# Gepeng18/Sentinel

Hardware: AMD Instinct MI355X
Metric: admission decisions/sec at 1M rules Zipf(1.1), 1/2/4/8 GPU; % HBM peak (higher is better)
Workload: dtype int64

## Files before the change

sentinel_amd/csrc/cluster.hip:

```cpp
#include "cluster.hpp"
#include "cluster_exact.hpp"
#include "cparam_exact.hpp"

#include <cstdio>
#include <cstdlib>

#include <algorithm>
#include <type_traits>

namespace sga {

namespace {

constexpr int kThreads = 256;
constexpr int kItems = 16;
constexpr int kTileElems = kThreads * kItems;

enum : uint8_t { RUN_FAST = 0, RUN_DONE = 1 };

__device__ __forceinline__ uint64_t lanemask_lt64(int lane) { return (1ULL << lane) - 1ULL; }

__device__ __forceinline__ HashEntry slot_lookup(const ClusterState &st, int64_t fid) {
    uint32_t h = (uint32_t)hash_flow_id(fid) & st.hmask;
    for (uint32_t probe = 0; probe <= st.hmask; ++probe) {
// ... 452 lines not shown
    const uint32_t f = pass_prefix(thr, P.isec, s0, a, n);
    uint32_t cpf = ri.cp_tot;
    if (f < n && ri.cp_tot > 0) cpf = prio_before(f);
    const uint32_t np_after = ri.cp_tot - cpf;
    uint32_t cw = 0;
    if (np_after > 0) {
        const int64_t w0 = c[CEV_WAITING] + waiting_others();
        const double latest = div_isec((double)(s0 + (int64_t)f * a), P.isec);
        const double lim = st.max_occupy_ratio * thr;
        const int64_t occ0 = o.occ_pass;
        uint32_t l2 = 0, h2 = np_after;
#pragma nounroll
        while (l2 < h2) {
            const uint32_t cc = l2 + ((h2 - l2) >> 1);
            const int64_t add = (int64_t)cc * a;
            const bool ok = (div_isec((double)(w0 + add), P.isec) <= lim) &&
                            (latest + (double)((int64_t)a + occ0 + add) - (double)head <= thr);
            if (ok) l2 = cc + 1;
            else h2 = cc;
        }
        cw = l2;
        if (cw > 0) {
            o.occ_pass += (int64_t)cw * a;
            o.occ_preq += cw;
            o.has_occ = 1;
            occ_dirty = true;
        }
    }
    const uint32_t nblk = n - f - cw;
    c[CEV_PASS] += (int64_t)f * a;
    c[CEV_PASS_REQUEST] += f;
    c[CEV_OCCUPIED_PASS] += (int64_t)cpf * a;
    c[CEV_WAITING] += (int64_t)cw * a;
    c[CEV_BLOCK] += (int64_t)nblk * a;
    c[CEV_BLOCK_REQUEST] += nblk;
    c[CEV_OCCUPIED_BLOCK] += (int64_t)(np_after - cw) * a;
    ro.s0 = s0;
    ro.thr = thr;
    ro.isec = P.isec;
    ro.f = f;
    ro.cpf = cpf;
    ro.cw = cw;
    ro.wait = (uint16_t)(1000 / P.S);
    ro.mode = RUN_FAST;
}

__device__ __forceinline__ void occ_transfer(int64_t (&c)[CEV_N], SlotOcc &o, bool &occ_dirty) {
    if (!o.has_occ) return;
    c[CEV_OCCUPIED_PASS] += o.occ_pass;
    c[CEV_PASS] += o.occ_pass;
    c[CEV_PASS_REQUEST] += o.occ_preq;
    o.occ_pass = 0;
    o.occ_preq = 0;
    o.has_occ = 0;
    occ_dirty = true;
}

template <class PrioBefore>
__device__ __forceinline__ bool run_compact(const ClusterState &st, const SlotParam &P, const Rec &R, double thr_in,
                                            bool hdr_thr, int64_t qbase, const RunIn &ri, PrioBefore prio_before,
                                            RunOut &ro, bool &wide) {
    int4 *lv = reinterpret_cast<int4 *>(R.ln());
    int4 L[8];
#pragma unroll
    for (int k = 0; k < 8; ++k) L[k] = lv[k];
    const uint64_t b0 = (uint64_t)i64_lo(L[LN_BASE / 4]);
    wide = (b0 & kLnWide) != 0;
    if (wide) return false;
    const int32_t a = ri.a;
    const int64_t q = qbase + ri.bd;
    if (a <= 0 || q < 0 || (int64_t)P.interval != (int64_t)P.S * (int64_t)P.W) return false;
    if (ri.cp_tot > 0 && (P.S <= 1 || 1000 / P.S <= 0)) return false;
    uint64_t b = b0;
    if (!(b & kLnBaseSet)) {
        const int64_t nb = ln_pick_base(q);
        if (!ln_base_fits(nb)) return false;
        b = (b & ~kLnBaseMask) | kLnBaseSet | (uint64_t)nb;
    }
    const int64_t base = ln_base(b);
    if (!ln_delta_fits(q, base)) return false;
    const uint32_t dq = ln_enc_delta(q, base);
    const int64_t qs = div_pos(q, P.S);
    const int cj = (int)(q - qs * P.S);
    const int jh = cj + 1 == P.S ? 0 : cj + 1;
    const double thr = hdr_thr ? f64_hi(L[LN_THR / 4]) : thr_in;
    auto valid = [&](uint32_t d) { return d != kLnNoBucket && !((int64_t)dq - (int64_t)d > (int64_t)P.S); };
    uint32_t dcur = kLnNoBucket, pcur = 0, dh = kLnNoBucket, ph = 0;
    int64_t bp = 0;
    auto take = [&](int jj, int d, int pv) {
        if (jj == cj) {
            dcur = (uint32_t)d;
            pcur = (uint32_t)pv;
        } else if (valid((uint32_t)d)) {
            bp += (int64_t)(uint32_t)pv;
        }
        if (jj == jh) {
            dh = (uint32_t)d;
            ph = (uint32_t)pv;
        }
    };
#pragma unroll
    for (int k = 0; k < kLnPairs / 2; ++k) {
        take(2 * k, L[k].x, L[k].y);
        take(2 * k + 1, L[k].z, L[k].w);
    }
    if (dcur != kLnNoBucket && dq < dcur) return false;
    const bool rot = dcur == kLnNoBucket || dq > dcur;
    int64_t c[CEV_N];
    SlotOcc o{(int64_t)(uint32_t)L[6].x, (int64_t)(uint32_t)L[6].y, (b & kLnHasOcc) ? 1 : 0, 0};
    bool occ_dirty = false;
    if (rot) {
#pragma unroll
        for (int k = 0; k < CEV_N; ++k) c[k] = 0;
        if (dcur != kLnNoBucket) occ_transfer(c, o, occ_dirty);
    } else {
        c[CEV_PASS] = (int64_t)pcur;
        if (ln_tag(b) == cj) {
            c[CEV_WAITING] = (int64_t)(uint32_t)L[6].z;
            c[CEV_BLOCK] = (int64_t)(uint32_t)L[6].w;
            c[CEV_PASS_REQUEST] = (int64_t)(uint32_t)L[7].x;
            c[CEV_BLOCK_REQUEST] = (int64_t)(uint32_t)L[7].y;
            c[CEV_OCCUPIED_PASS] = (int64_t)(uint32_t)L[7].z;
            c[CEV_OCCUPIED_BLOCK] = (int64_t)(uint32_t)L[7].w;
        } else {
            const int4 *cv = reinterpret_cast<const int4 *>(R.group(cj));
            const int4 c01 = cv[0], c23 = cv[1], c45 = cv[2];
            c[CEV_WAITING] = i64_lo(c01);
            c[CEV_BLOCK] = i64_hi(c01);
            c[CEV_PASS_REQUEST] = i64_lo(c23);
            c[CEV_BLOCK_REQUEST] = i64_hi(c23);
            c[CEV_OCCUPIED_PASS] = i64_lo(c45);
            c[CEV_OCCUPIED_BLOCK] = i64_hi(c45);
        }
    }
    const int64_t head = jh == cj ? c[CEV_PASS] : (valid(dh) ? (int64_t)ph : 0);
    auto waiting_others = [&]() {
        int64_t wv[kLnPairs], w0 = 0;
#pragma unroll
        for (int jj = 0; jj < kLnPairs; ++jj) wv[jj] = R.group(min(jj, P.S - 1))[0];
#pragma unroll
        for (int jj = 0; jj < kLnPairs; ++jj) {
            const uint32_t d = (uint32_t)((jj & 1) ? L[jj / 2].z : L[jj / 2].x);
            if (jj < P.S && jj != cj && valid(d)) w0 += wv[jj];
        }
        return w0;
    };
    run_decide(st, P, thr, ri, prio_before, waiting_others, bp, head, c, o, occ_dirty, ro);
    if (!ln_count_fits(c[CEV_PASS]) || !ln_count_fits(o.occ_pass) || !ln_count_fits(o.occ_preq)) return false;
    bool cfit = true;
#pragma unroll
    for (int k = 1; k < CEV_N; ++k) cfit = cfit && ln_count_fits(c[k]);
    uint64_t nb = ln_with_tag(b, cfit ? cj : -1);
    nb = o.has_occ ? (nb | kLnHasOcc) : (nb & ~kLnHasOcc);
    int4 pp = L[0];
#pragma unroll
    for (int k = 1; k < kLnPairs / 2; ++k)
        if (k == (cj >> 1)) pp = L[k];
    if (cj & 1) {
        pp.z = (int)dq;
        pp.w = (int)(uint32_t)c[CEV_PASS];
    } else {
        pp.x = (int)dq;
        pp.y = (int)(uint32_t)c[CEV_PASS];
    }
    lv[cj >> 1] = pp;
    if (nb != b0) lv[LN_BASE / 4] = make_int4((int)(uint32_t)nb, (int)(uint32_t)(nb >> 32), L[5].z, L[5].w);
    lv[6] = make_int4((int)(uint32_t)o.occ_pass, (int)(uint32_t)o.occ_preq, (int)(uint32_t)c[CEV_WAITING],
                      (int)(uint32_t)c[CEV_BLOCK]);
    lv[7] = make_int4((int)(uint32_t)c[CEV_PASS_REQUEST], (int)(uint32_t)c[CEV_BLOCK_REQUEST],
                      (int)(uint32_t)c[CEV_OCCUPIED_PASS], (int)(uint32_t)c[CEV_OCCUPIED_BLOCK]);
    int4 *cg = reinterpret_cast<int4 *>(R.group(cj));
    cg[0] = i4_of(c[CEV_WAITING], c[CEV_BLOCK]);
    cg[1] = i4_of(c[CEV_PASS_REQUEST], c[CEV_BLOCK_REQUEST]);
    cg[2] = i4_of(c[CEV_OCCUPIED_PASS], c[CEV_OCCUPIED_BLOCK]);
    return true;
}
static_assert(LN_BASE == 20 && LN_THR == 22 && LN_OCC == 24 && LN_CACHE == 26,
              "run_compact's pieces: 5 = (base word, threshold), 6 = (occupy counters, WAITING, BLOCK), 7 = the rest");

template <class PrioBefore>
__device__ __forceinline__ bool run_wide(const ClusterState &st, const SlotParam &P, const Rec &R, double thr_in,
                                         bool hdr_thr, int64_t qbase, const RunIn &ri, PrioBefore prio_before,
                                         RunOut &ro) {
    const int32_t a = ri.a;
    const int64_t q = qbase + ri.bd;
    const int64_t ws = q * P.W;
    const int64_t t0 = ws;
    const int64_t qs = div_pos(q, P.S);
    const int cj = (int)(q - qs * P.S);
    const int jh = cj + 1 == P.S ? 0 : cj + 1;
    const int4 *v = reinterpret_cast<const int4 *>(R.r);
    const int4 *hv = reinterpret_cast<const int4 *>(R.w_cache());
    const int4 *ov = reinterpret_cast<const int4 *>(&R.w_occ());
    const int4 o0 = ov[0], o1 = ov[1];
    int4 c01 = hv[0], c23 = hv[1], c45 = hv[2];
    const int4 meta = hv[3];
    const int4 cur = v[cj];
    const double thr = hdr_thr ? f64_hi(meta) : thr_in;
    auto valid = [&](int64_t w) { return w != kAbsent && !(t0 - w > (int64_t)P.interval); };
    int64_t bp = 0, hstart = kAbsent, hpass = 0;
    for (int jj = 0; jj < P.S; ++jj) {
        const int4 sp = v[jj];
        const int64_t w = i64_lo(sp), pv = i64_hi(sp);
        if (jj == jh) {
            hstart = w;
            hpass = pv;
        }
        if (jj != cj && valid(w)) bp += pv;
    }
    const int64_t old = i64_lo(cur);
    if (a <= 0 || (old != kAbsent && ws < old)) return false;
    if (ri.cp_tot > 0 && (P.S <= 1 || 1000 / P.S <= 0)) return false;
    const bool rot = old == kAbsent || ws > old;
    const bool tag_was_cur = i64_lo(meta) == old;
    if (!rot && !tag_was_cur) {
        const int4 *cv = reinterpret_cast<const int4 *>(R.group(cj));
        c01 = cv[0];
        c23 = cv[1];
        c45 = cv[2];
    }
    int64_t c[CEV_N];
    SlotOcc o{i64_lo(o0), i64_hi(o0), o1.x, o1.y};
    bool occ_dirty = false;
    if (rot) {
#pragma unroll
        for (int k = 0; k < CEV_N; ++k) c[k] = 0;
        if (old != kAbsent) occ_transfer(c, o, occ_dirty);
    } else {
        c[CEV_PASS] = i64_hi(cur);
        c[CEV_WAITING] = i64_lo(c01);
        c[CEV_BLOCK] = i64_hi(c01);
        c[CEV_PASS_REQUEST] = i64_lo(c23);
        c[CEV_BLOCK_REQUEST] = i64_hi(c23);
        c[CEV_OCCUPIED_PASS] = i64_lo(c45);
        c[CEV_OCCUPIED_BLOCK] = i64_hi(c45);
    }
    const int64_t head = jh == cj ? c[CEV_PASS] : (valid(hstart) ? hpass : 0);
    auto waiting_others = [&]() {
        int64_t w0 = 0;
#pragma nounroll
        for (int jj = 0; jj < P.S; ++jj)
            if (jj != cj && valid(R.w_start(jj))) w0 += R.cnt(CEV_WAITING, jj);
        return w0;
    };
    run_decide(st, P, thr, ri, prio_before, waiting_others, bp, head, c, o, occ_dirty, ro);
    const int64_t stv = rot ? ws : old;
    reinterpret_cast<int4 *>(R.r)[cj] = i4_of(stv, c[CEV_PASS]);
    c01 = i4_of(c[CEV_WAITING], c[CEV_BLOCK]);
    c23 = i4_of(c[CEV_PASS_REQUEST], c[CEV_BLOCK_REQUEST]);
    c45 = i4_of(c[CEV_OCCUPIED_PASS], c[CEV_OCCUPIED_BLOCK]);
    int4 *cg = reinterpret_cast<int4 *>(R.group(cj));
    cg[0] = c01;
    cg[1] = c23;
    cg[2] = c45;
    if (!rot && tag_was_cur) {
        int4 *ch = reinterpret_cast<int4 *>(R.w_cache());
        ch[0] = c01;
        ch[1] = c23;
        ch[2] = c45;
    }
    if (occ_dirty) {
        int4 *ow = reinterpret_cast<int4 *>(&R.w_occ());
        ow[0] = i4_of(o.occ_pass, o.occ_preq);
        ow[1] = make_int4(o.has_occ, o.pad, o1.z, o1.w);
    }
    return true;
}

__global__ __launch_bounds__(kRunThreads) void k_results(BatchScratch sc, const uint64_t *__restrict__ el,
                                                         uint32_t invalid_key, uint64_t *__restrict__ out) {
    const uint32_t nvalid = sc.counters[0];
    const uint32_t base = blockIdx.x * kTileElems;
    if (base >= nvalid) return;
    const int lane = threadIdx.x & 63, wave = threadIdx.x >> 6;
    if (base + wave * kWaveElems >= nvalid) return;
    const uint32_t e0 = base + threadIdx.x * kPerThread;
    uint64_t x[kPerThread];
    el_load_blk(el, e0, nvalid, invalid_key, x);
    const uint64_t first_prev = el_load(el, e0 - 1, e0 > 0 ? min(e0, nvalid) : 0, invalid_key);
    RAgg acc{0, 0, 0};
    {
        uint64_t px = first_prev;
#pragma unroll
        for (int k = 0; k < kPerThread; ++k) {
            const uint32_t e = e0 + k;
            const bool valid = e < nvalid;
            const bool h = valid && (e == 0 || el_runkey(x[k]) != el_runkey(px));
            acc = ragg_combine(acc, RAgg{h ? 1u : 0u, h ? 1u : 0u, valid ? el_prio(x[k]) : 0u});
            px = x[k];
        }
    }
    RAgg v = acc;
#pragma unroll
    for (int o = 1; o < 64; o <<= 1) {
        const RAgg y{shfl_up_u32(v.nh, o), shfl_up_u32(v.flag, o), shfl_up_u32(v.cnt, o)};
        if (lane >= o) v = ragg_combine(y, v);
    }
    RAgg excl{shfl_up_u32(v.nh, 1), shfl_up_u32(v.flag, 1), shfl_up_u32(v.cnt, 1)};
    if (lane == 0) excl = RAgg{0, 0, 0};
    RAgg run = ragg_combine(sc.wave_carry[blockIdx.x * kRunWaves + wave], excl);
    uint32_t rid[kPerThread], pcb[kPerThread];
    {
        uint64_t px = first_prev;
#pragma unroll
        for (int k = 0; k < kPerThread; ++k) {
            const uint32_t e = e0 + k;
            const bool h = e < nvalid && (e == 0 || el_runkey(x[k]) != el_runkey(px));
            const uint32_t p = e < nvalid ? el_prio(x[k]) : 0u;
            run = ragg_combine(run, RAgg{h ? 1u : 0u, h ? 1u : 0u, p});
            px = x[k];
            rid[k] = run.nh - 1;
            pcb[k] = run.cnt - p;
        }
    }
    constexpr int kResIlp = 8;
#pragma unroll
    for (int k0 = 0; k0 < kPerThread; k0 += kResIlp) {
        RunOut ro[kResIlp];
        uint32_t rs[kResIlp];
#pragma unroll
        for (int u = 0; u < kResIlp; ++u) {
            const int k = k0 + u;
            if (e0 + k < nvalid && (u == 0 || rid[k] != rid[k - 1])) {
                ro[u] = sc.run_out[rid[k]];
                rs[u] = sc.run_start[rid[k]];
            } else if (u > 0) {
                ro[u] = ro[u - 1];
                rs[u] = rs[u - 1];
            }
        }
#pragma unroll
        for (int u = 0; u < kResIlp; ++u) {
            const int k = k0 + u;
            const uint32_t e = e0 + k;
            if (e >= nvalid || ro[u].mode != RUN_FAST) continue;
            const uint32_t local = e - rs[u];
            const int32_t a = el_acq(x[k]);
            uint64_t res;
            if (local < ro[u].f) {
                const int64_t sum = ro[u].s0 + (int64_t)local * a;
                res = pack_result(TRS_OK, j_d2i(ro[u].thr - (double)sum / ro[u].isec - (double)a), 0);
            } else if (el_prio(x[k]) && pcb[k] - ro[u].cpf < ro[u].cw) {
                res = pack_result(TRS_SHOULD_WAIT, 0, (int32_t)ro[u].wait);
            } else {
                res = pack_result(TRS_BLOCKED, 0, 0);
            }
            out[el_idx(x[k])] = res;
        }
    }
}

constexpr int kFzThreads = 256, kFzPer = 4, kFzBlk = kFzThreads * kFzPer, kFzChunk = 2048;
constexpr int kFzDirect = 32;
constexpr int kFzLong = 512;
constexpr uint32_t kFzHuge = 2048;

#ifdef SGA_TEST_HOOKS
enum : int {
    CD_CHUNK = 0,
    CD_BIN,
    CD_BIN_LDS,
    CD_BIN_GLOBAL,
    CD_DIRECT,
    CD_WAVE,
    CD_WG,
    CD_REPLAY,
    CD_LISTFULL,
    CD_GLOBAL_REC,
    CD_CONT,
    CD_GALLOP,
    CD_PSEARCH,
    CD_COUNTER,
    CD_DROPPED,
    CD_HOTRUN,
    CD_HOTCW,
    CD_N
};
__device__ uint32_t g_cd[CD_N];
#define CD_COUNT(k) atomicAdd(&g_cd[k], 1u)
#else
#define CD_COUNT(k) ((void)0)
#endif

__device__ unsigned long long g_fz_phase[8];
__device__ __forceinline__ void fz_mark(int dbg, int ph, unsigned long long &t) {
    if (!(dbg & 16)) return;
    __syncthreads();
    const unsigned long long now = wall_clock64();
    if (threadIdx.x == 0 && ph > 0) atomicAdd(&g_fz_phase[ph - 1], now - t);
    if (threadIdx.x == 0 && ph == 3) atomicAdd(&g_fz_phase[7], 1ull);
    t = now;
}

struct FAgg {
    uint32_t hpos;
    uint32_t np;
    uint32_t hp;
    uint32_t flag;
    int32_t mn, mx;
};
__device__ __forceinline__ FAgg fagg_id() { return FAgg{0, 0, 0, 0, INT32_MAX, INT32_MIN}; }
__device__ __forceinline__ FAgg fagg_combine(const FAgg &a, const FAgg &b) {
    FAgg r;
    r.hpos = max(a.hpos, b.hpos);
    r.np = a.np + b.np;
    r.hp = b.flag ? a.np + b.hp : a.hp;
    r.flag = a.flag | b.flag;
    r.mn = b.flag ? b.mn : min(a.mn, b.mn);
    r.mx = b.flag ? b.mx : max(a.mx, b.mx);
    return r;
}
__device__ __forceinline__ FAgg fagg_shfl_up(const FAgg &v, int o) {
    return FAgg{shfl_up_u32(v.hpos, o), shfl_up_u32(v.np, o), shfl_up_u32(v.hp, o), shfl_up_u32(v.flag, o),
                __shfl_up(v.mn, o, 64), __shfl_up(v.mx, o, 64)};
}

template <int kCtrl, int kRowMask>
__device__ __forceinline__ FAgg fagg_dpp(const FAgg &v) {
    const FAgg id = fagg_id();
    auto mv = [](uint32_t old, uint32_t x) {
        return (uint32_t)__builtin_amdgcn_update_dpp((int)old, (int)x, kCtrl, kRowMask, 0xf, false);
    };
    return FAgg{mv(id.hpos, v.hpos), mv(id.np, v.np), mv(id.hp, v.hp), mv(id.flag, v.flag),
                (int32_t)mv((uint32_t)id.mn, (uint32_t)v.mn), (int32_t)mv((uint32_t)id.mx, (uint32_t)v.mx)};
}
template <int kCtrl, int kRowMask>
__device__ __forceinline__ void fagg_scan_step(FAgg &x) {
    x = fagg_combine(fagg_dpp<kCtrl, kRowMask>(x), x);
}

__device__ __forceinline__ FAgg fagg_block_excl(const FAgg &v, FAgg *total, FAgg *wtot) {
    const int lane = threadIdx.x & 63, wave = threadIdx.x >> 6;
    FAgg x = v;
    fagg_scan_step<0x111, 0xf>(x);
    fagg_scan_step<0x112, 0xf>(x);
    fagg_scan_step<0x114, 0xf>(x);
    fagg_scan_step<0x118, 0xf>(x);
    fagg_scan_step<0x142, 0xa>(x);
    fagg_scan_step<0x143, 0xc>(x);
    if (lane == 63) wtot[wave] = x;
    __syncthreads();
    FAgg pre = fagg_id(), t = fagg_id();
#pragma unroll
    for (int w = 0; w < kFzThreads / 64; ++w) {
        if (w < wave) pre = fagg_combine(pre, wtot[w]);
        t = fagg_combine(t, wtot[w]);
    }
    const FAgg ex = fagg_dpp<0x138, 0xf>(x);
    *total = t;
    __syncthreads();
    return fagg_combine(pre, ex);
}

__device__ __forceinline__ uint64_t match_lanes(uint32_t d, int bits, bool valid) {
    uint64_t peers = __ballot(valid);
    for (int b = 0; b < bits; ++b) {
        const bool bit = (d >> b) & 1u;
        const uint64_t bb = __ballot(bit);
        peers &= bit ? bb : ~bb;
    }
    return peers;
}
constexpr int kBinLds = 2560;
constexpr int kBoRounds = 12;
__device__ void bin_order(const uint64_t *__restrict__ in, uint64_t *es, uint32_t ebase, uint32_t B0, uint32_t B1,
                          int lb, uint32_t *pc, uint32_t *wsum) {
    const int lane = threadIdx.x & 63, wave = threadIdx.x >> 6;
    constexpr int kW = kFzThreads / 64;
    const uint32_t nd = 1u << lb, dm = nd - 1u;
    const uint64_t lt = lanemask_lt64(lane);
    for (uint32_t k = threadIdx.x; k < kW * nd; k += kFzThreads) pc[k] = 0;
    const uint32_t nb = B1 - B0;
    const uint32_t q = (((nb + kW - 1) / kW) + 63u) & ~63u;
    const uint32_t w0 = min(B1, B0 + (uint32_t)wave * q), w1 = min(B1, w0 + q);
    uint32_t *mine = pc + (uint32_t)wave * nd;
    uint64_t x[kBoRounds];
    auto load = [&](uint32_t c0) {
#pragma unroll
        for (int r = 0; r < kBoRounds; ++r) {
            const uint32_t p = c0 + (uint32_t)r * 64 + lane;
            x[r] = in[p < w1 ? p : (w0 < w1 ? w0 : B0)];
        }
    };
    const bool one = w1 - w0 <= (uint32_t)(kBoRounds * 64);
    __syncthreads();
    for (uint32_t c0 = w0; c0 < w1; c0 += kBoRounds * 64) {
        load(c0);
#pragma unroll
        for (int r = 0; r < kBoRounds; ++r) {
            if (c0 + (uint32_t)r * 64 >= w1) break;
            const bool valid = c0 + (uint32_t)r * 64 + lane < w1;
            const uint32_t d = el_slot(x[r]) & dm;
            const uint64_t peers = match_lanes(d, lb, valid);
            if (valid && (peers & lt) == 0) mine[d] += (uint32_t)__popcll(peers);
            __builtin_amdgcn_wave_barrier();
        }
    }
    __syncthreads();
    constexpr int kDpt = (1 << kPartMaxLow) / kFzThreads;
    uint32_t tot[kDpt], ts = 0;
#pragma unroll
    for (int k = 0; k < kDpt; ++k) {
        const uint32_t d = threadIdx.x * kDpt + k;
        uint32_t t = 0;
        if (d < nd)
            for (int w = 0; w < kW; ++w) t += pc[w * nd + d];
        tot[k] = t;
        ts += t;
    }
    uint32_t y = ts;
#pragma unroll
    for (int o = 1; o < 64; o <<= 1) {
        const uint32_t z = __shfl_up(y, o, 64);
        if (lane >= o) y += z;
    }
    if (lane == 63) wsum[wave] = y;
    __syncthreads();
    uint32_t pre = B0 + y - ts;
    for (int w = 0; w < wave; ++w) pre += wsum[w];
#pragma unroll
    for (int k = 0; k < kDpt; ++k) {
        const uint32_t d = threadIdx.x * kDpt + k;
        if (d < nd) {
            uint32_t run = pre;
            for (int w = 0; w < kW; ++w) {
                const uint32_t c = pc[w * nd + d];
                pc[w * nd + d] = run;
                run += c;
            }
        }
        pre += tot[k];
    }
    __syncthreads();
    for (uint32_t c0 = w0; c0 < w1; c0 += kBoRounds * 64) {
// ... 1663 lines not shown
    const uint32_t nh = hot_count(sc);
    for (uint32_t h = blockIdx.x * kThreads + threadIdx.x; h < nh; h += gridDim.x * kThreads) {
        const uint32_t slot = sc.hot_slot[h];
        sc.hot_of[slot] = kColdId;
        hot_fid_set(st, slot, kColdId);
    }
    __shared__ uint32_t bins[32];
    __shared__ unsigned long long best;
    if (threadIdx.x < 32) bins[threadIdx.x] = 0;
    if (threadIdx.x == 0) best = 0;
    __syncthreads();
    uint32_t ncold;
    const uint32_t ncand = hot_ncand(sc, ncold);
    unsigned long long mine = 0;
    for (uint32_t i = blockIdx.x * kThreads + threadIdx.x; i < ncand; i += gridDim.x * kThreads) {
        uint32_t slot, c;
        if (!hot_candidate(st, sc, i, ncold, hot_min, slot, c)) continue;
        atomicAdd(&bins[31 - __clz(c)], 1u);
        mine = max(mine, ((unsigned long long)c << 32) | slot);
    }
    if (mine) atomicMax(&best, mine);
    __syncthreads();
    if (threadIdx.x < 32 && bins[threadIdx.x]) atomicAdd(&sc.hot_ctl[8 + threadIdx.x], bins[threadIdx.x]);
    if (threadIdx.x == 0 && best) atomicMax(reinterpret_cast<unsigned long long *>(sc.hot_ctl + 4), best);
}

__global__ __launch_bounds__(kThreads) void k_hot_pick(ClusterState st, BatchScratch sc, uint32_t hot_min) {
    __shared__ uint32_t thr, wbest, bcnt[32], bbase[32], lcnt[32], gbase[32];
    if (threadIdx.x < 32) bcnt[threadIdx.x] = sc.hot_ctl[8 + threadIdx.x];
    __syncthreads();
    if (threadIdx.x == 0) {
        uint32_t cum = 0, t = 0xFFFFFFFFu;
        for (int b = 31; b >= 0; --b) {
            bbase[b] = cum;
            cum += bcnt[b];
            if (cum <= (uint32_t)kHot) t = 1u << b;
        }
        thr = max(t, max(hot_min, 1u));
        if (blockIdx.x == 0) sc.hot_ctl[7] = thr;
        const unsigned long long best = *reinterpret_cast<const unsigned long long *>(sc.hot_ctl + 4);
        wbest = best ? (uint32_t)st.param[(uint32_t)best].W : 0u;
    }
    __syncthreads();
    if (!wbest) return;
    uint32_t ncold;
    const uint32_t ncand = hot_ncand(sc, ncold);
    for (uint32_t r0 = blockIdx.x * kThreads; r0 < ncand; r0 += gridDim.x * kThreads) {
        if (threadIdx.x < 32) lcnt[threadIdx.x] = 0;
        __syncthreads();
        const uint32_t i = r0 + threadIdx.x;
        uint32_t slot = 0, c = 0, lo = 0;
        int b = -1;
        if (i < ncand && hot_candidate(st, sc, i, ncold, thr, slot, c) && (uint32_t)st.param[slot].W == wbest) {
            b = 31 - __clz(c);
            lo = atomicAdd(&lcnt[b], 1u);
        }
        __syncthreads();
        if (threadIdx.x < 32 && lcnt[threadIdx.x]) gbase[threadIdx.x] = atomicAdd(&sc.hot_ctl[64 + threadIdx.x], lcnt[threadIdx.x]);
        __syncthreads();
        if (b >= 0) {
            const uint32_t hid = bbase[b] + gbase[b] + lo;
            if (hid < (uint32_t)kHot) {
                sc.hot_next[hid] = slot;
                sc.hot_of[slot] = (uint16_t)hid;
                hot_fid_set(st, slot, (uint16_t)hid);
            }
        }
    }
}

constexpr int kFinThreads = 1024;
__global__ __launch_bounds__(kFinThreads) void k_hot_fin(ClusterState st, BatchScratch sc) {
    __shared__ uint32_t wsum[kFinThreads / 64];
    constexpr int kFinPer = kHot / kFinThreads;
    const int lane = threadIdx.x & 63, wave = threadIdx.x >> 6;
    uint32_t sl[kFinPer], cnt = 0;
#pragma unroll
    for (int k = 0; k < kFinPer; ++k) {
        sl[k] = sc.hot_next[threadIdx.x * kFinPer + k];
        cnt += sl[k] != kNoSlot;
    }
    uint32_t inc = cnt;
#pragma unroll
    for (int d = 1; d < 64; d <<= 1) {
        const uint32_t v = __shfl_up(inc, d);
        if (lane >= d) inc += v;
    }
    if (lane == 63) wsum[wave] = inc;
    __syncthreads();
    uint32_t off = 0, tot = 0;
    for (int w = 0; w < kFinThreads / 64; ++w) {
        off += w < wave ? wsum[w] : 0u;
        tot += wsum[w];
    }
    uint32_t hid = off + inc - cnt;
#pragma unroll
    for (int k = 0; k < kFinPer; ++k) {
        const uint32_t at = threadIdx.x * kFinPer + k;
        if (sl[k] == kNoSlot) continue;
        sc.hot_slot[hid] = sl[k];
        if (hid != at) {
            sc.hot_of[sl[k]] = (uint16_t)hid;
            hot_fid_set(st, sl[k], (uint16_t)hid);
        }
        sc.hot_next[at] = kNoSlot;
        ++hid;
    }
    if (threadIdx.x == 0) {
        const unsigned long long best = *reinterpret_cast<const unsigned long long *>(sc.hot_ctl + 4);
        sc.hot_ctl[2] = best ? (uint32_t)st.param[(uint32_t)best].W : 1u;
        sc.hot_ctl[0] = tot;
        sc.hot_ctl[4] = 0;
        sc.hot_ctl[5] = 0;
        sc.hot_ctl[6] = 0;
    }
    if (threadIdx.x < 32) {
        sc.hot_ctl[8 + threadIdx.x] = 0;
        sc.hot_ctl[64 + threadIdx.x] = 0;
    }
    if (threadIdx.x < CTL_WORDS) {
        sc.counters_last[threadIdx.x] = sc.counters[threadIdx.x];
        sc.counters[threadIdx.x] = 0;
    }
}

__global__ void k_hot_reset(ClusterState st, BatchScratch sc, uint32_t nslots_cap) {
    for (uint32_t i = blockIdx.x * blockDim.x + threadIdx.x; i < nslots_cap; i += gridDim.x * blockDim.x)
        sc.hot_of[i] = kColdId;
    if (st.dkey)
        for (uint32_t i = blockIdx.x * blockDim.x + threadIdx.x; i < st.dense_n; i += gridDim.x * blockDim.x)
            st.dkey[i] = st.dense[i] == ~0u ? kDkNone : st.dense[i];
    for (uint32_t i = blockIdx.x * blockDim.x + threadIdx.x; i < (uint32_t)kHot; i += gridDim.x * blockDim.x)
        sc.hot_next[i] = kNoSlot;
    if (blockIdx.x == 0 && threadIdx.x < kHotCtlWords) sc.hot_ctl[threadIdx.x] = 0;
    if (blockIdx.x == 0 && threadIdx.x == 0) {
        *sc.tmax_all = 0;
        sc.pstart[kPartBins + 1] = 0;
    }
}

__global__ void k_metric_sums(ClusterState st, uint32_t s, int64_t now, int64_t *out7) {
    if (threadIdx.x != 0 || blockIdx.x != 0) return;
    const SlotParam P = st.param[s];
    cur_window(st, P, s, now);
    for (int k = 0; k < CEV_N; ++k) out7[k] = values_sum(st, P, now, k);
}

__global__ __launch_bounds__(kThreads) void k_cluster_nodes(ClusterState st, const int64_t *__restrict__ slot_fid,
                                                            int64_t now, sga_cluster_metric_node *out, uint32_t cap,
                                                            uint32_t *count) {
    __shared__ uint32_t wbase[kThreads / 64];
    __shared__ uint32_t base;
    const uint32_t s = blockIdx.x * kThreads + threadIdx.x;
    const bool act = s < st.nslots && st.param[s].active;
    sga_cluster_metric_node m{};
    if (act) {
        const SlotParam P = st.param[s];
        m.flow_id = slot_fid[s];
        cur_window(st, P, s, now);
        const Rec R = rec_of(st, P);
        int64_t sb = 0, sp = 0;
        if (P.S <= kLnPairs && !R.wide()) {
            int4 pr[kLnPairs / 2 + 1];
            int64_t bl[kLnPairs];
#pragma unroll
            for (int k = 0; k < kLnPairs / 2 + 1; ++k) pr[k] = reinterpret_cast<const int4 *>(R.ln())[k];
#pragma unroll
            for (int j = 0; j < kLnPairs; ++j) bl[j] = R.cnt(CEV_BLOCK, min(j, P.S - 1));
            const int64_t base = ln_base((uint64_t)i64_lo(pr[LN_BASE / 4]));
#pragma unroll
            for (int j = 0; j < kLnPairs; ++j) {
                const uint32_t d = (uint32_t)((j & 1) ? pr[j / 2].z : pr[j / 2].x);
                const uint32_t pv = (uint32_t)((j & 1) ? pr[j / 2].w : pr[j / 2].y);
                const int64_t w = ln_dec_bucket(d, base) * (int64_t)P.W;
                if (j < P.S && d != kLnNoBucket && !(now - w > (int64_t)P.interval)) {
                    sp += (int64_t)pv;
                    sb += bl[j];
                }
            }
        } else {
            sb = values_sum(st, P, now, CEV_BLOCK);
            sp = values_sum(st, P, now, CEV_PASS);
        }
        m.block_qps = (double)sb / P.isec;
        m.pass_qps = (double)sp / P.isec;
        m.timestamp = now;
    }
    const int lane = threadIdx.x & 63, wave = threadIdx.x >> 6;
    const uint64_t bm = __ballot(act);
    if (lane == 0) wbase[wave] = (uint32_t)__popcll(bm);
    __syncthreads();
    if (threadIdx.x == 0) {
        uint32_t t = 0;
        for (int w = 0; w < kThreads / 64; ++w) {
            const uint32_t c = wbase[w];
            wbase[w] = t;
            t += c;
        }
        base = t ? atomicAdd(count, t) : 0u;
    }
    __syncthreads();
    if (act) {
        const uint32_t k = base + wbase[wave] + (uint32_t)__popcll(bm & lanemask_lt64(lane));
        if (k < cap) out[k] = m;
    }
}

__global__ void k_init_slots(ClusterState st, const uint32_t *slots, uint32_t n) {
    const uint32_t i = blockIdx.x * kThreads + threadIdx.x;
    if (i >= n) return;
    const uint32_t s = slots[i];
    const SlotParam P = st.param[s];
    rec_of(st, P).init(P.thr);
}

__global__ void k_rec_thr(ClusterState st, uint32_t n) {
    const uint32_t s = blockIdx.x * kThreads + threadIdx.x;
    if (s >= n) return;
    const SlotParam P = st.param[s];
    if (P.S <= 0) return;
    rec_of(st, P).set_thr(P.thr);
}


constexpr int kLimW = 100, kLimN = 10, kLimInterval = 1000;

template <class RuleParam>
__global__ __launch_bounds__(kThreads) void k_lim_flag(const RuleParam *param, const uint64_t *__restrict__ el,
                                                       uint32_t n, uint32_t invalid, int32_t ns,
                                                       uint32_t *__restrict__ flag) {
    const uint32_t i = blockIdx.x * kThreads + threadIdx.x;
    if (i >= n) return;
    const uint32_t k = el_slot(el[i]);
    flag[i] = (k != invalid && param[k].ns == ns) ? 1u : 0u;
}

__global__ __launch_bounds__(kThreads) void k_lim_compact(const uint32_t *__restrict__ flag,
                                                          const uint32_t *__restrict__ pos, uint32_t n,
                                                          uint32_t *__restrict__ list, uint32_t *counters) {
    const uint32_t i = blockIdx.x * kThreads + threadIdx.x;
    if (i >= n) return;
    if (flag[i]) list[pos[i]] = i;
    if (i == n - 1) counters[4] = pos[i] + flag[i];
}

__global__ __launch_bounds__(kThreads) void k_lim_heads(const uint32_t *__restrict__ list,
                                                        const uint32_t *__restrict__ ts_off, int64_t ts_base,
                                                        uint32_t n, const uint32_t *counters,
                                                        uint32_t *__restrict__ head) {
    const uint32_t j = blockIdx.x * kThreads + threadIdx.x;
    if (j >= n) return;
    const uint32_t m = counters[4];
    uint32_t h = 0;
    if (j < m) {
        const int64_t b = (ts_base + (int64_t)ts_off[list[j]]) / kLimW;
        h = (j == 0 || b != (ts_base + (int64_t)ts_off[list[j - 1]]) / kLimW) ? 1u : 0u;
    }
    head[j] = h;
}

__global__ __launch_bounds__(kThreads) void k_lim_starts(const uint32_t *__restrict__ head,
                                                         const uint32_t *__restrict__ ridx, uint32_t n,
                                                         uint32_t *counters, uint32_t *__restrict__ rstart) {
    const uint32_t j = blockIdx.x * kThreads + threadIdx.x;
    const uint32_t m = counters[4];
    if (j >= m || j >= n) return;
    if (head[j]) rstart[ridx[j]] = j;
    if (j == m - 1) counters[5] = ridx[j] + head[j];
}

__global__ void k_lim_walk(NsLimiterDev *L, double qps_allowed, const uint32_t *__restrict__ list,
                           const uint32_t *__restrict__ rstart, const uint32_t *counters,
                           const uint32_t *__restrict__ ts_off, int64_t ts_base, uint32_t *__restrict__ rpass) {
    if (threadIdx.x || blockIdx.x) return;
    const uint32_t m = counters[4], R = counters[5];
    for (uint32_t r = 0; r < R && m; ++r) {
        const uint32_t j0 = rstart[r], j1 = r + 1 < R ? rstart[r + 1] : m;
        const int64_t nr = (int64_t)(j1 - j0);
        const int64_t t = ts_base + (int64_t)ts_off[list[j0]];
        const int idx = (int)((t / kLimW) % kLimN);
        const int64_t ws = t - t % kLimW;
        bool detached = false;
        if (L->start[idx] == kAbsent || ws > L->start[idx]) {
            L->start[idx] = ws;
            L->cnt[idx] = 0;
        } else if (ws < L->start[idx]) {
            detached = true;
        }
        int64_t others = 0;
        for (int k = 0; k < kLimN; ++k) {
            if (!detached && k == idx) continue;
            if (L->start[k] != kAbsent && !(t - L->start[k] > kLimInterval)) others += L->cnt[k];
        }
        int64_t pass;
        if (detached) {
            pass = ((double)others / 1.0 + 1 <= qps_allowed) ? nr : 0;
        } else {
            const int64_t c0 = L->cnt[idx];
            int64_t lo = 0, hi = nr;
            while (lo < hi) {
                const int64_t mid = lo + ((hi - lo) >> 1);
                if ((double)(others + c0 + mid) / 1.0 + 1 <= qps_allowed) lo = mid + 1;
                else hi = mid;
            }
            pass = lo;
            L->cnt[idx] = c0 + pass;
        }
        rpass[r] = (uint32_t)pass;
    }
}

__global__ __launch_bounds__(kThreads) void k_lim_apply(const uint32_t *__restrict__ list,
                                                        const uint32_t *__restrict__ head,
                                                        const uint32_t *__restrict__ ridx,
                                                        const uint32_t *__restrict__ rstart,
                                                        const uint32_t *__restrict__ rpass, const uint32_t *counters,
                                                        uint32_t n, uint32_t invalid, uint64_t *__restrict__ el,
                                                        uint64_t *__restrict__ out) {
    const uint32_t j = blockIdx.x * kThreads + threadIdx.x;
    const uint32_t m = counters[4];
    if (j >= m || j >= n) return;
    const uint32_t r = ridx[j] + head[j] - 1;
    if (j - rstart[r] >= rpass[r]) {
        const uint32_t i = list[j];
        el[i] = (uint64_t)invalid << kSlotShift;
        out[i] = pack_result(TRS_TOO_MANY_REQUEST, 0, 0);
    }
}

__global__ void k_lim_init(NsLimiterDev *L) {
// ... 997 lines not shown
    }
}

void cparam_sum(const CParamState &st, uint32_t slot, int64_t value, int64_t now, int64_t *d_out, hipStream_t s) {
    hipLaunchKernelGGL(k_psum, dim3(1), dim3(64), 0, s, st, slot, value, now, d_out);
}

void cparam_top_values(const CParamState &st, uint32_t slot, int64_t now, uint32_t number, int64_t *d_list,
                       uint32_t *d_count, int64_t *d_val, double *d_qps, uint32_t *d_n, hipStream_t s) {
    hipLaunchKernelGGL(k_pwindow, dim3(1), dim3(64), 0, s, st, slot, now);
    SGA_HIP_CHECK(hipMemsetAsync(d_count, 0, sizeof(uint32_t), s));
    const uint32_t nk = st.kmask + 1;
    hipLaunchKernelGGL(k_ptop_collect, dim3((nk + kThreads - 1) / kThreads), dim3(kThreads), 0, s, st, slot, now,
                       d_list, d_count);
    hipLaunchKernelGGL(k_ptop_select, dim3(1), dim3(1024), 0, s, st, slot, d_list, d_count, number, d_val, d_qps,
                       d_n);
}

void cparam_init_rule(const CParamState &st, uint32_t slot, hipStream_t s) {
    hipLaunchKernelGGL(k_pinit_rule, dim3(1), dim3(64), 0, s, st, slot);
}

void cluster_metric_nodes(const ClusterState &st, const int64_t *slot_fid, int64_t now, void *out, uint32_t cap,
                          uint32_t *count, hipStream_t s) {
    SGA_HIP_CHECK(hipMemsetAsync(count, 0, 4, s));
    if (st.nslots == 0) return;
    hipLaunchKernelGGL(k_cluster_nodes, dim3((st.nslots + kThreads - 1) / kThreads), dim3(kThreads), 0, s, st,
                       slot_fid, now, (sga_cluster_metric_node *)out, cap, count);
}

__global__ __launch_bounds__(kThreads) void k_ts_offsets(const int32_t *__restrict__ ts, int64_t lo,
                                                         uint32_t *__restrict__ off, uint32_t n) {
    const uint32_t i = blockIdx.x * kThreads + threadIdx.x;
    if (i < n) off[i] = (uint32_t)((int64_t)ts[i] - lo);
}

void cluster_ts_offsets(const int32_t *ts, int64_t lo, uint32_t *off, uint32_t n, hipStream_t s) {
    if (n) hipLaunchKernelGGL(k_ts_offsets, dim3((n + kThreads - 1) / kThreads), dim3(kThreads), 0, s, ts, lo, off, n);
}

__global__ __launch_bounds__(kThreads) void k_ts_minmax(const int64_t *__restrict__ ts, uint32_t n, int64_t *mm) {
    int64_t lo = INT64_MAX, hi = INT64_MIN;
    for (uint32_t i = blockIdx.x * kThreads + threadIdx.x; i < n; i += gridDim.x * kThreads) {
        const int64_t t = ts[i];
        lo = min(lo, t);
        hi = max(hi, t);
    }
    lo = wave_min_i64(lo);
    hi = wave_max_i64(hi);
    if ((threadIdx.x & 63) == 0) {
        atomicMin((long long *)&mm[0], (long long)lo);
        atomicMax((long long *)&mm[1], (long long)hi);
    }
}

__global__ void k_ts_minmax_init(int64_t *mm) {
    if (threadIdx.x == 0) {
        mm[0] = INT64_MAX;
        mm[1] = INT64_MIN;
    }
}

void cluster_ts_minmax(const int64_t *ts, uint32_t n, int64_t *minmax, hipStream_t s) {
    hipLaunchKernelGGL(k_ts_minmax_init, dim3(1), dim3(64), 0, s, minmax);
    if (n) hipLaunchKernelGGL(k_ts_minmax, dim3(std::min<uint32_t>((n + kThreads - 1) / kThreads, 2048)), dim3(kThreads), 0, s,
                              ts, n, minmax);
}

__global__ __launch_bounds__(kThreads) void k_ts_offsets64(const int64_t *__restrict__ ts, int64_t lo,
                                                           uint32_t *__restrict__ off, uint32_t n) {
    const uint32_t i = blockIdx.x * kThreads + threadIdx.x;
    if (i < n) off[i] = (uint32_t)(ts[i] - lo);
}

void cluster_ts_offsets64(const int64_t *ts, int64_t lo, uint32_t *off, uint32_t n, hipStream_t s) {
    if (n) hipLaunchKernelGGL(k_ts_offsets64, dim3((n + kThreads - 1) / kThreads), dim3(kThreads), 0, s, ts, lo, off, n);
}

void cluster_init_limiter(NsLimiterDev *d, hipStream_t s) {
    hipLaunchKernelGGL(k_lim_init, dim3(1), dim3(64), 0, s, d);
}

__global__ __launch_bounds__(kThreads) void k_rls_expand(const uint32_t *__restrict__ off, uint32_t nreq,
                                                         const int64_t *__restrict__ dfid,
                                                         const int32_t *__restrict__ hits,
                                                         const uint32_t *__restrict__ ts_off, int64_t *fid_out,
                                                         int32_t *acq_out, uint32_t *ts_out) {
    const uint32_t r = blockIdx.x * kThreads + threadIdx.x;
    if (r >= nreq) return;
    const int32_t h = hits[r];
    const int32_t a = h <= 0 ? 1 : h;
    const uint32_t t = ts_off[r];
    for (uint32_t d = off[r]; d < off[r + 1]; ++d) {
        fid_out[d] = h < 0 ? 0 : dfid[d];
        acq_out[d] = a;
        ts_out[d] = t;
    }
}

__global__ __launch_bounds__(kThreads) void k_rls_finish(const uint32_t *__restrict__ off, uint32_t nreq,
                                                         const int32_t *__restrict__ hits,
                                                         const uint64_t *__restrict__ res, int8_t *desc_status,
                                                         int32_t *desc_rem, int32_t *code) {
    const uint32_t r = blockIdx.x * kThreads + threadIdx.x;
    if (r >= nreq) return;
    const bool skip = hits[r] < 0;
    bool blocked = false;
    for (uint32_t d = off[r]; d < off[r + 1]; ++d) {
        const int8_t stt = skip ? (int8_t)TRS_NO_RULE_EXISTS : (int8_t)(res[d] >> 48);
        blocked |= stt != TRS_OK && stt != TRS_NO_RULE_EXISTS;
        if (desc_status) desc_status[d] = stt;
        if (desc_rem) desc_rem[d] = skip ? 0 : (int32_t)(uint32_t)res[d];
    }
    code[r] = skip ? -1 : (blocked ? 2 : 1);
}

void rls_expand(const uint32_t *off, uint32_t nreq, const int64_t *dfid, const int32_t *hits, const uint32_t *ts_off,
                int64_t *fid_out, int32_t *acq_out, uint32_t *ts_out, hipStream_t s) {
    if (!nreq) return;
    hipLaunchKernelGGL(k_rls_expand, dim3((nreq + kThreads - 1) / kThreads), dim3(kThreads), 0, s, off, nreq, dfid,
                       hits, ts_off, fid_out, acq_out, ts_out);
}

void rls_finish(const uint32_t *off, uint32_t nreq, const int32_t *hits, const uint64_t *res, int8_t *desc_status,
                int32_t *desc_rem, int32_t *code, hipStream_t s) {
    if (!nreq) return;
    hipLaunchKernelGGL(k_rls_finish, dim3((nreq + kThreads - 1) / kThreads), dim3(kThreads), 0, s, off, nreq, hits,
                       res, desc_status, desc_rem, code);
}

void cluster_metric_sums(const ClusterState &st, uint32_t slot, int64_t now, int64_t *d_out7, hipStream_t s) {
    hipLaunchKernelGGL(k_metric_sums, dim3(1), dim3(64), 0, s, st, slot, now, d_out7);
}

void cluster_init_slots(const ClusterState &st, const uint32_t *d_slots, uint32_t n, hipStream_t s) {
    if (n == 0) return;
    hipLaunchKernelGGL(k_init_slots, dim3((n + kThreads - 1) / kThreads), dim3(kThreads), 0, s, st, d_slots, n);
}

void cluster_sync_rec_thr(const ClusterState &st, uint32_t n, hipStream_t s) {
    hipLaunchKernelGGL(k_rec_thr, dim3((n + kThreads - 1) / kThreads), dim3(kThreads), 0, s, st, n);
}

}

#ifdef SGA_TEST_HOOKS
extern "C" int sga_test_cluster_dispatch(uint32_t *out, size_t n) {
    if (!out || n < (size_t)sga::CD_N) return -1;
    if (hipDeviceSynchronize() != hipSuccess) return -1;
    if (hipMemcpyFromSymbol(out, HIP_SYMBOL(sga::g_cd), sizeof(uint32_t) * sga::CD_N, 0, hipMemcpyDeviceToHost) != hipSuccess)
        return -1;
    return (int)sga::CD_N;
}
#endif
```

sentinel_amd/csrc/cluster_exact.hpp:

```cpp
#pragma once
#include <hip/hip_runtime.h>

#include "cluster.hpp"
#include "cluster_line.hpp"

namespace sga {

enum : int8_t { TRS_BAD_REQUEST = -4, TRS_TOO_MANY_REQUEST = -2, TRS_FAIL = -1, TRS_OK = 0, TRS_BLOCKED = 1,
                TRS_SHOULD_WAIT = 2, TRS_NO_RULE_EXISTS = 3 };

__device__ __forceinline__ uint64_t pack_result(int8_t status, int32_t remaining, int32_t wait) {
    return (uint64_t)(uint32_t)remaining | ((uint64_t)(uint16_t)(int16_t)wait << 32) |
           ((uint64_t)(uint8_t)status << 48);
}

constexpr int kOccWords = 4;
static_assert(sizeof(SlotOcc) <= kOccWords * 8, "occupy state fits its words");
constexpr int kCacheWords = 6;
__host__ __device__ constexpr int rec_hdr_words(int S) { return 2 * S + kOccWords + kCacheWords + 2; }
__host__ __device__ constexpr uint32_t rec_units(int S) {
    return 2u + (((uint32_t)(8 * S + 12 + 7) / 8 + 1u) & ~1u);
}
static_assert(rec_hdr_words(10) == 32 && rec_units(10) == 14, "S = 10: line, two-line header, 896-byte record");
static_assert(kLnWords64 * 8 == 128, "the decision line is one 128-byte line");
struct Rec {
    int64_t *r;
    int S;
    int32_t W;
    __device__ __forceinline__ uint32_t *ln() const { return reinterpret_cast<uint32_t *>(r - kLnWords64); }
    __device__ __forceinline__ uint64_t &bw() const { return *reinterpret_cast<uint64_t *>(ln() + LN_BASE); }
    __device__ __forceinline__ bool wide() const { return (bw() & kLnWide) != 0; }
    __device__ __forceinline__ int64_t &w_start(int j) const { return r[2 * j]; }
    __device__ __forceinline__ int64_t &w_pass(int j) const { return r[2 * j + 1]; }
    __device__ __forceinline__ SlotOcc &w_occ() const { return *reinterpret_cast<SlotOcc *>(r + 2 * S); }
    __device__ __forceinline__ int64_t *w_cache() const { return r + 2 * S + kOccWords; }
    __device__ __forceinline__ int64_t &w_tag() const { return r[2 * S + kOccWords + kCacheWords]; }
    __device__ __forceinline__ double &w_thr() const {
        return *reinterpret_cast<double *>(r + 2 * S + kOccWords + kCacheWords + 1);
    }
    __device__ __forceinline__ int64_t *group(int j) const { return r + rec_hdr_words(S) + 6 * j; }
    __device__ __forceinline__ int64_t &cnt(int ev, int j) const {
        if (ev == CEV_WAITING) return group(j)[0];
        return group(j)[ev];
    }
    __device__ inline void widen() const {
        const uint64_t b = bw();
        if (b & kLnWide) return;
        const uint32_t *l = ln();
        const int64_t base = ln_base(b);
        for (int j = 0; j < S && j < kLnPairs; ++j) {
            const uint32_t d = l[2 * j];
            w_start(j) = d == kLnNoBucket ? kAbsent : ln_dec_bucket(d, base) * (int64_t)W;
            w_pass(j) = (int64_t)l[2 * j + 1];
        }
        w_occ() = SlotOcc{(int64_t)l[LN_OCC], (int64_t)l[LN_OCC + 1], (b & kLnHasOcc) ? 1 : 0, 0};
        const int tg = ln_tag(b);
        if (tg >= 0) {
            for (int k = 0; k < kCacheWords; ++k) w_cache()[k] = (int64_t)l[LN_CACHE + k];
            w_tag() = w_start(tg);
        } else {
            w_tag() = kAbsent;
        }
        bw() = b | kLnWide;
    }
    __device__ inline int64_t start(int j) const {
        const uint64_t b = bw();
        if (b & kLnWide) return w_start(j);
        const uint32_t d = ln()[2 * j];
        return d == kLnNoBucket ? kAbsent : ln_dec_bucket(d, ln_base(b)) * (int64_t)W;
    }
    __device__ inline void set_start(int j, int64_t ws) const {
        uint64_t b = bw();
        if (!(b & kLnWide)) {
            const int64_t q = ws / W;
            bool fits = ws >= 0 && q * (int64_t)W == ws;
            if (fits && !(b & kLnBaseSet)) {
                const int64_t nb = ln_pick_base(q);
                fits = ln_base_fits(nb);
                if (fits) b = (b & ~kLnBaseMask) | kLnBaseSet | (uint64_t)nb;
            }
            fits = fits && ln_delta_fits(q, ln_base(b));
            if (fits) {
                if (ln_tag(b) == j) b = ln_with_tag(b, -1);
                bw() = b;
                ln()[2 * j] = ln_enc_delta(q, ln_base(b));
                return;
            }
            widen();
        }
        w_start(j) = ws;
    }
    __device__ inline int64_t pass(int j) const { return wide() ? w_pass(j) : (int64_t)ln()[2 * j + 1]; }
    __device__ inline void set_pass(int j, int64_t v) const {
        if (!wide()) {
            if (ln_count_fits(v)) {
                ln()[2 * j + 1] = (uint32_t)v;
                return;
            }
            widen();
        }
        w_pass(j) = v;
    }
    __device__ inline SlotOcc occ() const {
        const uint64_t b = bw();
        if (b & kLnWide) return w_occ();
        return SlotOcc{(int64_t)ln()[LN_OCC], (int64_t)ln()[LN_OCC + 1], (b & kLnHasOcc) ? 1 : 0, 0};
    }
    __device__ inline void set_occ(const SlotOcc &o) const {
        const uint64_t b = bw();
        if (!(b & kLnWide)) {
            if (ln_count_fits(o.occ_pass) && ln_count_fits(o.occ_preq)) {
                ln()[LN_OCC] = (uint32_t)o.occ_pass;
                ln()[LN_OCC + 1] = (uint32_t)o.occ_preq;
                bw() = o.has_occ ? (b | kLnHasOcc) : (b & ~kLnHasOcc);
                return;
            }
            widen();
        }
        w_occ() = o;
    }
    __device__ inline void cache_drop(int j) const {
        const uint64_t b = bw();
        if (b & kLnWide) {
            if (w_tag() == w_start(j)) w_tag() = kAbsent;
        } else if (ln_tag(b) == j) {
            bw() = ln_with_tag(b, -1);
        }
    }
    __device__ inline void set_cache(int j, const int64_t (&g)[kCacheWords]) const {
        const uint64_t b = bw();
        if (b & kLnWide) {
            for (int k = 0; k < kCacheWords; ++k) w_cache()[k] = g[k];
            w_tag() = w_start(j);
            return;
        }
        bool fits = true;
        for (int k = 0; k < kCacheWords; ++k) fits = fits && ln_count_fits(g[k]);
        if (fits)
            for (int k = 0; k < kCacheWords; ++k) ln()[LN_CACHE + k] = (uint32_t)g[k];
        bw() = ln_with_tag(b, fits ? j : -1);
    }
    __device__ inline double thr() const { return *reinterpret_cast<const double *>(ln() + LN_THR); }
    __device__ inline void set_thr(double v) const {
        *reinterpret_cast<double *>(ln() + LN_THR) = v;
        w_thr() = v;
    }
    __device__ inline void init(double thr_v) const {
        uint32_t *l = ln();
        for (int j = 0; j < kLnPairs; ++j) {
            l[2 * j] = kLnNoBucket;
            l[2 * j + 1] = 0;
        }
        bw() = S > kLnPairs ? kLnWide : 0ull;
        for (int k = LN_OCC; k < 2 * kLnWords64; ++k) l[k] = 0;
        for (int j = 0; j < S; ++j) {
            w_start(j) = kAbsent;
            w_pass(j) = 0;
            for (int k = 0; k < 6; ++k) group(j)[k] = 0;
        }
        w_occ() = SlotOcc{0, 0, 0, 0};
        w_tag() = kAbsent;
        set_thr(thr_v);
    }
};

__device__ __forceinline__ Rec rec_of(const ClusterState &st, const SlotParam &P) {
    return Rec{st.rec + (size_t)P.boff * 8 + kLnWords64, P.S, (int32_t)P.W};
}

struct WinRef {
    int j;
    bool detached;
};

__device__ __forceinline__ void bucket_zero(const Rec &R, int j) {
#pragma unroll
    for (int k = 1; k < CEV_N; ++k) R.cnt(k, j) = 0;
    R.set_pass(j, 0);
}

__device__ inline WinRef cur_window(const ClusterState &st, const SlotParam &P, uint32_t s, int64_t t) {
    const Rec R = rec_of(st, P);
    const int j = (int)((t / P.W) % P.S);
    const int64_t ws = t - t % P.W;
    const int64_t old = R.start(j);
    if (old == kAbsent) {
        R.set_start(j, ws);
        bucket_zero(R, j);
        return WinRef{j, false};
    }
    if (ws == old) return WinRef{j, false};
    if (ws > old) {
        R.set_start(j, ws);
        bucket_zero(R, j);
        SlotOcc o = R.occ();
        if (o.has_occ) {
            R.cnt(CEV_OCCUPIED_PASS, j) += o.occ_pass;
            R.set_pass(j, R.pass(j) + o.occ_pass);
            o.occ_pass = 0;
            R.cnt(CEV_PASS_REQUEST, j) += o.occ_preq;
            o.occ_preq = 0;
            o.has_occ = 0;
            R.set_occ(o);
        }
        return WinRef{j, false};
    }
    return WinRef{j, true};
}

__device__ inline int64_t values_sum(const ClusterState &st, const SlotParam &P, int64_t t, int ev) {
    const Rec R = rec_of(st, P);
    int64_t s = 0;
    for (int j = 0; j < P.S; ++j) {
        const int64_t w = R.start(j);
        if (w != kAbsent && !(t - w > (int64_t)P.interval)) s += ev == CEV_PASS ? R.pass(j) : R.cnt(ev, j);
    }
    return s;
}

__device__ __forceinline__ double get_avg(const ClusterState &st, const SlotParam &P, uint32_t s, int64_t t, int ev) {
    cur_window(st, P, s, t);
    return (double)values_sum(st, P, t, ev) / P.isec;
}

__device__ __forceinline__ void metric_add(const ClusterState &st, const SlotParam &P, uint32_t s, int64_t t, int ev,
                                           int64_t n) {
    const WinRef w = cur_window(st, P, s, t);
    if (w.detached) return;
    const Rec R = rec_of(st, P);
    if (ev == CEV_PASS) {
        R.set_pass(w.j, R.pass(w.j) + n);
    } else {
        R.cnt(ev, w.j) += n;
        R.cache_drop(w.j);
    }
}

__device__ __forceinline__ int64_t head_pass(const ClusterState &st, const SlotParam &P, int64_t t) {
    const Rec R = rec_of(st, P);
    const int j = (int)(((t + P.W) / P.W) % P.S);
    const int64_t w = R.start(j);
    return (w != kAbsent && !(t - w > (int64_t)P.interval)) ? R.pass(j) : 0;
}

__device__ inline uint64_t request_exact(const ClusterState &st, uint32_t s, int64_t t, int32_t a, bool p, int simple) {
    const SlotParam P = st.param[s];
    const double thr = simple ? P.thr_simple : P.thr;
    const double latest = get_avg(st, P, s, t, CEV_PASS);
    const double rem = thr - latest - (double)a;
    if (rem >= 0) {
        metric_add(st, P, s, t, CEV_PASS, a);
        metric_add(st, P, s, t, CEV_PASS_REQUEST, 1);
        if (p) metric_add(st, P, s, t, CEV_OCCUPIED_PASS, a);
        return pack_result(TRS_OK, j_d2i(rem), 0);
    }
    if (p) {
        const double occupy_avg = get_avg(st, P, s, t, CEV_WAITING);
        if (occupy_avg <= st.max_occupy_ratio * thr) {
            const double latest2 = get_avg(st, P, s, t, CEV_PASS);
            const int64_t head = head_pass(st, P, t);
            const Rec R = rec_of(st, P);
            SlotOcc o = R.occ();
            if (latest2 + (double)((int64_t)a + o.occ_pass) - (double)head <= thr) {
                o.occ_pass += a;
                o.occ_preq += 1;
                o.has_occ = 1;
                R.set_occ(o);
                metric_add(st, P, s, t, CEV_WAITING, a);
                const int32_t wait = 1000 / P.S;
                if (wait > 0) return pack_result(TRS_SHOULD_WAIT, 0, wait);
            }
        }
    }
    metric_add(st, P, s, t, CEV_BLOCK, a);
    metric_add(st, P, s, t, CEV_BLOCK_REQUEST, 1);
    if (p) metric_add(st, P, s, t, CEV_OCCUPIED_BLOCK, a);
    return pack_result(TRS_BLOCKED, 0, 0);
}


}
```

sentinel_amd/csrc/cluster_line.hpp:

```cpp
#pragma once
#include <stdint.h>

#if defined(__HIPCC__) || defined(__CUDACC__)
#define SGA_LN_HD __host__ __device__ inline
#else
#define SGA_LN_HD inline
#endif

namespace sga {

constexpr int kLnPairs = 10;
constexpr int kLnWords64 = 16;
constexpr int kLnBaseBits = 47;
constexpr uint64_t kLnBaseMask = (1ull << kLnBaseBits) - 1;
constexpr uint64_t kLnBaseSet = 1ull << 56;
constexpr int kLnTagShift = 57;
constexpr uint64_t kLnTagMask = 0xFull << kLnTagShift;
constexpr uint64_t kLnTagValid = 1ull << 61;
constexpr uint64_t kLnHasOcc = 1ull << 62;
constexpr uint64_t kLnWide = 1ull << 63;
constexpr uint32_t kLnNoBucket = 0xFFFFFFFFu;
constexpr int64_t kLnMaxDelta = 0xFFFFFFFEll;
constexpr int64_t kLnMaxCount = 0xFFFFFFFFll;
constexpr int64_t kLnBaseMargin = 1ll << 16;
static_assert(kLnPairs <= 16, "the tag's bucket index has four bits");
static_assert((kLnBaseMask & (kLnBaseSet | kLnTagMask | kLnTagValid | kLnHasOcc | kLnWide)) == 0 &&
                  (kLnBaseSet & kLnTagMask) == 0 && (kLnTagMask & kLnTagValid) == 0,
              "the flags lie above the base and do not overlap");
static_assert(2 * kLnPairs + 2 + 2 + 2 + 6 == 32, "the line is exactly 32 words");

enum : int { LN_BASE = 20, LN_THR = 22, LN_OCC = 24, LN_CACHE = 26 };

SGA_LN_HD bool ln_base_fits(int64_t q) { return q >= 0 && q <= (int64_t)kLnBaseMask; }
SGA_LN_HD int64_t ln_pick_base(int64_t q) { return q > kLnBaseMargin ? q - kLnBaseMargin : 0; }
SGA_LN_HD int64_t ln_base(uint64_t bw) { return (int64_t)(bw & kLnBaseMask); }
SGA_LN_HD bool ln_delta_fits(int64_t q, int64_t base) {
    return q >= base && q - base <= kLnMaxDelta;
}
SGA_LN_HD uint32_t ln_enc_delta(int64_t q, int64_t base) { return (uint32_t)(uint64_t)(q - base); }
SGA_LN_HD int64_t ln_dec_bucket(uint32_t d, int64_t base) { return base + (int64_t)d; }
SGA_LN_HD bool ln_count_fits(int64_t v) { return v >= 0 && v <= kLnMaxCount; }
SGA_LN_HD int ln_tag(uint64_t bw) { return (bw & kLnTagValid) ? (int)((bw & kLnTagMask) >> kLnTagShift) : -1; }
SGA_LN_HD uint64_t ln_with_tag(uint64_t bw, int j) {
    bw &= ~(kLnTagMask | kLnTagValid);
    return j < 0 ? bw : (bw | kLnTagValid | ((uint64_t)j << kLnTagShift));
}

}
```

Before: 24.61 billion.

## Flag lines with nonzero block counts and skip block reads in metric snapshot

```diff
diff --git a/sentinel_amd/csrc/cluster.hip b/sentinel_amd/csrc/cluster.hip
--- a/sentinel_amd/csrc/cluster.hip
+++ b/sentinel_amd/csrc/cluster.hip
@@ -628,6 +628,7 @@
     for (int k = 1; k < CEV_N; ++k) cfit = cfit && ln_count_fits(c[k]);
     uint64_t nb = ln_with_tag(b, cfit ? cj : -1);
     nb = o.has_occ ? (nb | kLnHasOcc) : (nb & ~kLnHasOcc);
+    if (c[CEV_BLOCK] != 0) nb |= kLnAnyBlock;
     int4 pp = L[0];
 #pragma unroll
     for (int k = 1; k < kLnPairs / 2; ++k)
@@ -854,8 +855,12 @@
 };
 __device__ uint32_t g_cd[CD_N];
 #define CD_COUNT(k) atomicAdd(&g_cd[k], 1u)
+enum : int { SN_COMPACT = 0, SN_FLAGGED, SN_CLEARED, SN_N };
+__device__ uint32_t g_sn[SN_N];
+#define SN_COUNT(k) atomicAdd(&g_sn[k], 1u)
 #else
 #define CD_COUNT(k) ((void)0)
+#define SN_COUNT(k) ((void)0)
 #endif
 
 __device__ unsigned long long g_fz_phase[8];
@@ -2825,22 +2830,33 @@
     __shared__ uint32_t wbase[kThreads / 64];
     __shared__ uint32_t base;
     const uint32_t s = blockIdx.x * kThreads + threadIdx.x;
-    const bool act = s < st.nslots && st.param[s].active;
+    SlotParam P{};
+    if (s < st.nslots) {
+        if (st.uni_S) {
+            P.S = st.uni_S;
+            P.W = st.uni_W;
+            P.interval = st.uni_iv;
+            P.isec = st.uni_iv / 1000.0;
+            P.boff = s * rec_units(st.uni_S);
+            P.active = st.param[s].active;
+        } else {
+            P = st.param[s];
+        }
+    }
+    const bool act = P.active != 0;
     sga_cluster_metric_node m{};
     if (act) {
-        const SlotParam P = st.param[s];
         m.flow_id = slot_fid[s];
         cur_window(st, P, s, now);
         const Rec R = rec_of(st, P);
         int64_t sb = 0, sp = 0;
         if (P.S <= kLnPairs && !R.wide()) {
             int4 pr[kLnPairs / 2 + 1];
-            int64_t bl[kLnPairs];
 #pragma unroll
             for (int k = 0; k < kLnPairs / 2 + 1; ++k) pr[k] = reinterpret_cast<const int4 *>(R.ln())[k];
-#pragma unroll
-            for (int j = 0; j < kLnPairs; ++j) bl[j] = R.cnt(CEV_BLOCK, min(j, P.S - 1));
-            const int64_t base = ln_base((uint64_t)i64_lo(pr[LN_BASE / 4]));
+            const uint64_t b = (uint64_t)i64_lo(pr[LN_BASE / 4]);
+            const int64_t base = ln_base(b);
+            uint32_t vm = 0;
 #pragma unroll
             for (int j = 0; j < kLnPairs; ++j) {
                 const uint32_t d = (uint32_t)((j & 1) ? pr[j / 2].z : pr[j / 2].x);
@@ -2848,7 +2864,23 @@
                 const int64_t w = ln_dec_bucket(d, base) * (int64_t)P.W;
                 if (j < P.S && d != kLnNoBucket && !(now - w > (int64_t)P.interval)) {
                     sp += (int64_t)pv;
-                    sb += bl[j];
+                    vm |= 1u << j;
+                }
+            }
+            SN_COUNT(SN_COMPACT);
+            if (b & kLnAnyBlock) {
+                SN_COUNT(SN_FLAGGED);
+                int64_t bl[kLnPairs], any = 0;
+#pragma unroll
+                for (int j = 0; j < kLnPairs; ++j) bl[j] = R.cnt(CEV_BLOCK, min(j, P.S - 1));
+#pragma unroll
+                for (int j = 0; j < kLnPairs; ++j) {
+                    any |= bl[j];
+                    if ((vm >> j) & 1u) sb += bl[j];
+                }
+                if (any == 0) {
+                    R.bw() = b & ~kLnAnyBlock;
+                    SN_COUNT(SN_CLEARED);
                 }
             }
         } else {
@@ -4152,4 +4184,14 @@
         return -1;
     return (int)sga::CD_N;
 }
+
+extern "C" int sga_test_cluster_snapshot(uint32_t *out, size_t n) {
+    if (!out || n < (size_t)sga::SN_N) return -1;
+    if (hipDeviceSynchronize() != hipSuccess) return -1;
+    const uint32_t z[sga::SN_N] = {};
+    if (hipMemcpyFromSymbol(out, HIP_SYMBOL(sga::g_sn), sizeof(z), 0, hipMemcpyDeviceToHost) != hipSuccess ||
+        hipMemcpyToSymbol(HIP_SYMBOL(sga::g_sn), z, sizeof(z), 0, hipMemcpyHostToDevice) != hipSuccess)
+        return -1;
+    return (int)sga::SN_N;
+}
 #endif
diff --git a/sentinel_amd/csrc/cluster_exact.hpp b/sentinel_amd/csrc/cluster_exact.hpp
--- a/sentinel_amd/csrc/cluster_exact.hpp
+++ b/sentinel_amd/csrc/cluster_exact.hpp
@@ -138,7 +138,11 @@
         for (int k = 0; k < kCacheWords; ++k) fits = fits && ln_count_fits(g[k]);
         if (fits)
             for (int k = 0; k < kCacheWords; ++k) ln()[LN_CACHE + k] = (uint32_t)g[k];
-        bw() = ln_with_tag(b, fits ? j : -1);
+        bw() = ln_with_tag(b, fits ? j : -1) | (g[CEV_BLOCK] != 0 ? kLnAnyBlock : 0ull);
+    }
+    __device__ inline void mark_block() const {
+        const uint64_t b = bw();
+        if (!(b & kLnAnyBlock)) bw() = b | kLnAnyBlock;
     }
     __device__ inline double thr() const { return *reinterpret_cast<const double *>(ln() + LN_THR); }
     __device__ inline void set_thr(double v) const {
@@ -233,6 +237,7 @@
     } else {
         R.cnt(ev, w.j) += n;
         R.cache_drop(w.j);
+        if (ev == CEV_BLOCK && n != 0) R.mark_block();
     }
 }
 
diff --git a/sentinel_amd/csrc/cluster_line.hpp b/sentinel_amd/csrc/cluster_line.hpp
--- a/sentinel_amd/csrc/cluster_line.hpp
+++ b/sentinel_amd/csrc/cluster_line.hpp
@@ -13,6 +13,7 @@
 constexpr int kLnWords64 = 16;
 constexpr int kLnBaseBits = 47;
 constexpr uint64_t kLnBaseMask = (1ull << kLnBaseBits) - 1;
+constexpr uint64_t kLnAnyBlock = 1ull << 55;
 constexpr uint64_t kLnBaseSet = 1ull << 56;
 constexpr int kLnTagShift = 57;
 constexpr uint64_t kLnTagMask = 0xFull << kLnTagShift;
@@ -24,8 +25,9 @@
 constexpr int64_t kLnMaxCount = 0xFFFFFFFFll;
 constexpr int64_t kLnBaseMargin = 1ll << 16;
 static_assert(kLnPairs <= 16, "the tag's bucket index has four bits");
-static_assert((kLnBaseMask & (kLnBaseSet | kLnTagMask | kLnTagValid | kLnHasOcc | kLnWide)) == 0 &&
-                  (kLnBaseSet & kLnTagMask) == 0 && (kLnTagMask & kLnTagValid) == 0,
+static_assert((kLnBaseMask & (kLnAnyBlock | kLnBaseSet | kLnTagMask | kLnTagValid | kLnHasOcc | kLnWide)) == 0 &&
+                  (kLnBaseSet & kLnTagMask) == 0 && (kLnTagMask & kLnTagValid) == 0 &&
+                  (kLnAnyBlock & (kLnBaseSet | kLnTagMask | kLnTagValid | kLnHasOcc | kLnWide)) == 0,
               "the flags lie above the base and do not overlap");
 static_assert(2 * kLnPairs + 2 + 2 + 2 + 6 == 32, "the line is exactly 32 words");
 
```

New measurement: 24.44 billion. Within noise of the previous version (-0.7%).
